# TritonDataCenter/dragnet

Measured on AMD Instinct MI355X. Metric: NDJSON records/sec (whole node), krill filter + 2-field breakdown (req.method,res.statusCode), higher is better.
Workload: dtype uint8; 1 GPU; model=dn scan: filter eq(req.method,GET) + breakdown req.method,res.statusCode, global_batch=4743501, seq_len=226, parallelism=dp1

## Files before the change

dragnet_amd/engine/gpu.py:

```python

import os
import stat
from types import SimpleNamespace

import numpy as np

from . import capacity, decode, xpose
from . import plan as planmod
from .chunks import _pad, choose_chunk_bytes, frame_files
from .decode import (
    C_DS_FAILEDEVAL, C_DS_FILTERED, C_GLOBAL_N, C_INVALID_JSON, C_LINES,
    C_OVERFLOW, C_PARSED, CM_AGG_IN, CM_BADDATE, CM_FAILEDEVAL,
    CM_FILTER_IN, CM_FILTERED, CM_N, CM_NONNUMERIC, CM_TIME_OUT, CM_UNDEF)
from .xpose import _build_xpose_layout


def _env_int(name, default):
    try:
        return int(os.environ.get(name, default))
    except ValueError:
        return default


def first_guess_slots():
# ... 287 lines not shown
    def overflowed(self):
        return int(self.counters[C_OVERFLOW].item()) > 0


    def scan_files(self, files):
        cap = self.eng.chunk_bytes
        if self._pinned is None:
            try:
                total = sum(os.stat(p).st_size for p in files)
            except OSError:
                total = 0
            cap = choose_chunk_bytes(total, cap,
                                     "DRAGNET_CHUNK_MB" in os.environ)
        pins = self._ensure_file_staging(cap)
        evs = [None, None]

        def wait(i):
            if evs[i] is not None:
                evs[i].synchronize()
                evs[i] = None

        frames = frame_files(files, [memoryview(p.numpy()) for p in pins],
                             cap, wait, _env_int("DRAGNET_READERS", 24))
        try:
            for i, n in frames:
                evs[i] = self._run_pinned(pins[i], n)
        finally:
            frames.close()

    def _ensure_file_staging(self, cap):
        torch = self.t
        if self._files is None:
            if self._pinned is None:
                self._ensure_buffers(_pad(cap))
            self._files = SimpleNamespace(
                pins=[self._pinned, torch.empty(
                    self._pinned.numel(), dtype=torch.uint8,
                    pin_memory=True)],
                copy_stream=torch.cuda.Stream(device=self.eng.device),
                dev=[self._dev_data, torch.empty_like(self._dev_data)],
                done=[torch.cuda.Event(), torch.cuda.Event()],
                idx=0)
        return self._files.pins

    def _run_pinned(self, pin, n):
        torch = self.t
        f = self._files
        padded = self._pad_pinned(pin, n)
        idx = f.idx
        f.idx ^= 1
        dev_data = f.dev[idx]
        main = torch.cuda.current_stream(self.eng.device)
        cs = f.copy_stream
        cs.wait_event(f.done[idx])
        ev = torch.cuda.Event()
        with torch.cuda.stream(cs):
            dev_data[:padded].copy_(pin[:padded], non_blocking=True)
            ev.record(cs)
        main.wait_event(ev)
        self._submit(dev_data, 0, n)
        f.done[idx].record(main)
        return ev


    def stage_resident(self, buf, n_slices=None):
        torch = self.t
        if n_slices is None:
            n_slices = _env_int("DRAGNET_SLICES", 6)
        n = len(buf)
        self._ensure_buffers(_pad(n))
        pin = self._pinned
        pin[:n] = torch.frombuffer(bytearray(buf), dtype=torch.uint8)
        padded = self._pad_pinned(pin, n)

        bounds = sorted({0, n} | {buf.rfind(b"\n", 0, n * k // n_slices) + 1
                                  for k in range(1, n_slices)})
        slices = list(zip(bounds, bounds[1:]))
        self._pool = p = SimpleNamespace(
            n=n, padded=padded, slices=slices,
            copy_stream=torch.cuda.Stream(device=self.eng.device),
            evs=[torch.cuda.Event() for _ in slices],
            dev_pp=torch.empty_like(self._dev_data),
            pass_done=[torch.cuda.Event(), torch.cuda.Event()],
            idx=0, pos=[])

        self._dev_data[:padded].copy_(pin[:padded])
        for (s, e) in slices:
            pos, nlines = self._index(self._dev_data, s, e)
            p.pos.append(
                (pos[:int(nlines.item())].clone(), nlines.clone()))

    def scan_resident(self, h2d=True):
        torch = self.t
        p = self._pool
        padded = p.padded
        dev_data = self._dev_data
        pin = self._pinned
        main = torch.cuda.current_stream(self.eng.device)
        if h2d:
            idx = p.idx
            p.idx ^= 1
            dev_data = self._dev_data if idx == 0 else p.dev_pp
            ev_done = p.pass_done[idx]
            p.copy_stream.wait_event(ev_done)
            with torch.cuda.stream(p.copy_stream):
                for k, (s, e) in enumerate(p.slices):
                    s16 = s & ~15
                    e16 = min((e + 15) & ~15, padded)
                    dev_data[s16:e16].copy_(pin[s16:e16],
                                            non_blocking=True)
                    p.evs[k].record(p.copy_stream)
        for k, (s, e) in enumerate(p.slices):
            if h2d:
                main.wait_event(p.evs[k])
                self._submit(dev_data, s, e)
            else:
                self._submit(dev_data, s, e, p.pos[k])
        if h2d:
            ev_done.record(main)


    def stage_xpose(self, buf=None):
        gran = _env_int("DRAGNET_XGRAN", 64)
        if gran not in (32, 64, 128):
            raise ValueError("DRAGNET_XGRAN must be 32, 64 or 128")
        if os.environ.get("DRAGNET_XPOSE_HOST") == "1":
            self._x = xpose.build_on_host(self.t, buf, gran,
                                          self.eng.device)
            return
        if self._pool is None:
            if buf is None:
                raise ValueError("no resident pool to transpose")
            self.stage_resident(buf)
        pos, nlines = self._index(self._dev_data, 0, self._pool.n)
        self._x = xpose.build_on_device(self.t, self.eng.ops,
                                        self._dev_data, pos, nlines, gran)

    def scan_xpose(self):
        self.state.scan_xpose(*self._x)

    def make_graph(self, h2d=True, xpose=False):
        torch = self.t

        def pass_():
            self.reset()
            if xpose:
                self.scan_xpose()
            else:
                self.scan_resident(h2d=h2d)

        try:
            pass_()
            torch.cuda.synchronize(self.eng.device)
            g = torch.cuda.CUDAGraph()
            with torch.cuda.graph(g):
                pass_()
            torch.cuda.synchronize(self.eng.device)
            return g
        except Exception:
            return None

    def reset(self):
        self.state.reset()
        if self.planner is not None:
            self.planner.occ = dict.fromkeys(self.planner.names, 0)


    def finalize(self, queries):
        return self.decode_extracted(self.extract_async(queries),
                                     queries)

    def extract_async(self, queries):
        h = self.state.extract_all()
        h["ev"] = self.t.cuda.Event()
        h["ev"].record()
        return h

    def decode_extracted(self, h, queries):
        torch = self.t
        if self._fin_stream is None:
            self._fin_stream = torch.cuda.Stream(device=self.eng.device)
        with torch.cuda.stream(self._fin_stream):
            self._fin_stream.wait_event(h["ev"])
            host = {"cnt": h["cnt"].cpu().numpy()}
            host.update(self._fetch_dicts(h))
            host["aggs"] = []
            for k_full, c_full, out_n in h["aggs"][:len(queries)]:
                n_out = min(int(out_n.item()), k_full.shape[0])
                host["aggs"].append((k_full[:n_out].cpu().numpy(),
                                     c_full[:n_out].cpu().numpy()))
        return decode.decode_snapshot(host, queries, self.cplan)

    @staticmethod
    def _fetch_dicts(h):
        n_str = int(h["n_str"].item())
        n_num = int(h["n_num"].item())
        host = {"n_str": n_str, "n_num": n_num}
        if n_str:
            host["str_off"] = h["str_off"][:n_str].cpu().numpy()
            host["str_len"] = h["str_len"][:n_str].cpu().numpy()
            used = int(h["used"].item())
            host["blob"] = h["blob"][:used].cpu().numpy()
# ... 8 lines not shown
```

dragnet_amd/ops/hip/common.h:

```cpp
#pragma once
#if defined(__HIPCC__)
#include <hip/hip_runtime.h>
#endif
#include <cstddef>
#include <cstdint>
#include "hd.h"

namespace dn {

constexpr int MAX_FIELDS = 24;
constexpr int MAX_DEPTH  = 64;
constexpr int SLOT_DEPTH = 12;
constexpr int MAX_KEY    = 8;
constexpr int MAX_SYNTH  = 8;
constexpr int PRED_STACK = 8;

enum PredOp : int32_t {
  OP_AND = 0, OP_OR = 1,
  OP_EQ = 2, OP_NE = 3, OP_LT = 4, OP_LE = 5, OP_GT = 6, OP_GE = 7,
  OP_TRUE = 8,
};

enum ConstKind : int32_t { CONST_NUM = 0, CONST_STR = 1, CONST_NULL = 2 };

// ... 22 lines not shown
enum CounterSlot : int {
  C_LINES = 0,
  C_INVALID_JSON = 1,
  C_PARSED = 2,
  C_DS_FILTERED = 3,
  C_DS_FAILEDEVAL = 4,
  C_OVERFLOW = 5,
  C_GLOBAL_N = 8,
  CM_FILTER_IN = 0, CM_FILTERED = 1, CM_FAILEDEVAL = 2,
  CM_UNDEF = 3, CM_BADDATE = 4, CM_TIME_OUT = 5,
  CM_AGG_IN = 6, CM_NONNUMERIC = 7,
  CM_N = 8,
};

constexpr uint32_t SLOT_EMPTY = 0, SLOT_CLAIMED = 1, SLOT_READY = 2;

struct AggTable {
  uint32_t* state;
  uint32_t* keys;
  double*   count;
  uint32_t  nslots;
  double*   partial;
  uint32_t  prows;
  uint32_t  pad_;
};

struct StrDict {
  uint32_t* state;
  uint64_t* hash;
  uint32_t* id;
  uint32_t* off;
  uint32_t* len;
  uint32_t  nslots;
  uint8_t*  data;
  uint32_t  data_cap;
  uint32_t* data_used;
  uint32_t* next_id;
};

struct NumDict {
  uint32_t* state;
  uint64_t* bits;
  uint32_t* id;
  uint32_t  nslots;
  uint32_t* next_id;
};


struct PlanView {
  const uint64_t* field_sigs;
  int nf;
  const int32_t* comp_slot;
  int nf_match;
  uint64_t sig_bloom;
  const int32_t* prog_nodes;
  const int32_t* prog_bounds;
  const int32_t* const_meta;
  const double*  const_dvals;
  const uint8_t* const_bytes;
  const int32_t* synth_slots;
  int ns;
  const int32_t* metric_rows;
  const int32_t* synth_req;
  const int32_t* bd_rows;
  const double*  bd_steps;
  int nm;
  int value_slot;
  int fields_slot;
  uint64_t fields_parent_sig;
};

struct ScanArgs {
  const uint8_t* data;
  const uint32_t* nl_pos;
  const uint32_t* nlines_ptr;
  uint32_t pos_cap;
  uint32_t first_start;
  uint32_t tile_cap;
  PlanView P;
  AggTable* tables;
  StrDict sdict;
  NumDict ndict;
  unsigned long long* counters;
  int data_format_skinner;
  const uint8_t* xdata;
  const unsigned long long* xwave_base;
  const uint32_t* xrec_len;
  uint32_t xn_slots;
};

}
```

dragnet_amd/ops/hip/ext.hip:

```cpp

#include <torch/extension.h>
#include <cstdlib>
#include <cstring>
#include <c10/hip/HIPStream.h>

#include "scan_kernels.hip"

namespace dn {

namespace {

#define CHECK_GPU(t) TORCH_CHECK((t).is_cuda(), #t " must be on GPU")

constexpr size_t LDS_MAX = 160 * 1024;

hipStream_t current_stream() {
  return c10::hip::getCurrentHIPStream().stream();
}

template <class... KArgs, class... Args>
void launch(const char* what, void (*kernel)(KArgs...), dim3 grid,
            dim3 block, size_t lds, Args&&... args) {
  hipLaunchKernelGGL(kernel, grid, block, lds, current_stream(),
                     std::forward<Args>(args)...);
  hipError_t err = hipGetLastError();
  TORCH_CHECK(err == hipSuccess, what, " launch failed: ",
              hipGetErrorString(err));
}

constexpr uint32_t GRID_CAP = 2048;

uint32_t grid_for(uint64_t n) {
  return (uint32_t)std::min<uint64_t>((n + BLOCK - 1) / BLOCK, GRID_CAP);
}

int env_int(const char* name, int dflt) {
  const char* v = getenv(name);
  return v ? atoi(v) : dflt;
}

size_t lds_bytes(int64_t nf, int64_t nm, int64_t ns, bool columnar) {
  return LdsLayout((int)nf, (int)nm, columnar ? 0 : (int)ns, !columnar)
      .total;
}

using ScanKernel = void (*)(ScanArgs);

ScanKernel linear_kernel(int mw) {
  switch (mw) {
    case 2: return scan_kernel_mw<2>;
    case 3: return scan_kernel_mw<3>;
    case 4: return scan_kernel_mw<4>;
    case 5: return scan_kernel_mw<5>;
    case 6: return scan_kernel_mw<6>;
    default: return scan_kernel;
  }
}

ScanKernel xpose_kernel(int mw, int xg) {
  if (xg == 32) return scan_kernel_x<4, 5>;
  if (xg == 128) return scan_kernel_x<4, 7>;
  switch (mw) {
    case 2: return scan_kernel_x<2, 6>;
    case 3: return scan_kernel_x<3, 6>;
    case 5: return scan_kernel_x<5, 6>;
    default: return scan_kernel_x<4, 6>;
  }
}

}

void newline_index(torch::Tensor data, int64_t start, int64_t n,
                   torch::Tensor seg_scratch,
                   torch::Tensor pos_out, torch::Tensor total_out) {
  CHECK_GPU(data);
  int64_t span = n - (start & ~(int64_t)15);
  uint32_t nseg = (uint32_t)((span + NL_SEG - 1) / NL_SEG);
  TORCH_CHECK((int64_t)nseg <= seg_scratch.numel(),
              "seg_scratch too small");
  if (span <= 0) {
    total_out.zero_();
    return;
  }
  const uint8_t* d = (const uint8_t*)data.data_ptr();
  uint32_t* segs = (uint32_t*)seg_scratch.data_ptr();
  uint32_t blocks = (nseg + 3) / 4;
// ... 17 lines not shown
  for (int f = 0; f < nf; f++) {
    d[f].kind = (int32_t)kinds[f];
    d[f].num = kinds[f] == COL_NUM ? (const double*)nums[f].data_ptr()
                                   : nullptr;
    d[f].soff = (kinds[f] == COL_STR || kinds[f] == COL_CODED)
                    ? (const uint32_t*)soffs[f].data_ptr()
                    : nullptr;
    d[f].slen = kinds[f] == COL_STR ? (const uint32_t*)slens[f].data_ptr()
                                    : nullptr;
  }
  return out;
}

void xpose_build(torch::Tensor data, torch::Tensor sstart,
                 torch::Tensor slen, torch::Tensor wbase,
                 int64_t n_slots, int64_t gran_log, torch::Tensor xb) {
  CHECK_GPU(data);
  CHECK_GPU(xb);
  uint32_t nw = (uint32_t)(n_slots >> 6);
  TORCH_CHECK(wbase.numel() >= (long)nw + 1, "wbase needs nw+1 rows");
  uint32_t blocks = (nw + 3) / 4;
  launch("xpose_build", xpose_build_kernel, dim3(blocks), dim3(256), 0,
         (const uint8_t*)data.data_ptr(),
         (const uint32_t*)sstart.data_ptr(),
         (const uint32_t*)slen.data_ptr(),
         (const unsigned long long*)wbase.data_ptr(),
         (uint32_t)n_slots, (int)gran_log, (uint8_t*)xb.data_ptr());
}

class ScanState {
 public:
  ScanState(py::dict plan, int64_t agg_slots, int64_t dict_slots,
            int64_t dict_data_bytes, bool dense)
      : dense_(dense) {
    auto ptr = [&](py::dict& d, const char* key) {
      owned_.push_back(py::cast<torch::Tensor>(d[key]));
      return owned_.back().data_ptr();
    };
    PlanView& P = args_.P;
    P.field_sigs = (const uint64_t*)ptr(plan, "field_sigs");
    P.nf = (int)owned_.back().numel();
    P.comp_slot = (const int32_t*)ptr(plan, "comp_slot");
    P.nf_match = py::cast<int>(plan["nf_match"]);
    P.sig_bloom = (uint64_t)py::cast<int64_t>(plan["sig_bloom"]);
    P.prog_nodes = (const int32_t*)ptr(plan, "prog_nodes");
    P.prog_bounds = (const int32_t*)ptr(plan, "prog_bounds");
    P.const_meta = (const int32_t*)ptr(plan, "const_meta");
    P.const_dvals = (const double*)ptr(plan, "const_dvals");
    P.const_bytes = (const uint8_t*)ptr(plan, "const_bytes");
    P.synth_slots = (const int32_t*)ptr(plan, "synth_slots");
    P.ns = py::cast<int>(plan["n_synth"]);
    P.metric_rows = (const int32_t*)ptr(plan, "metric_rows");
    P.nm = (int)(owned_.back().numel() / 8);
    P.synth_req = (const int32_t*)ptr(plan, "synth_req");
    P.bd_rows = (const int32_t*)ptr(plan, "bd_rows");
    P.bd_steps = (const double*)ptr(plan, "bd_steps");
    P.value_slot = py::cast<int>(plan["value_slot"]);
    P.fields_slot = py::cast<int>(plan["fields_slot"]);
    P.fields_parent_sig =
        (uint64_t)py::cast<int64_t>(plan["fields_parent_sig"]);
    args_.data_format_skinner = py::cast<bool>(plan["skinner"]) ? 1 : 0;

    for (auto& t : owned_) CHECK_GPU(t);
    device_ = owned_.front().device();

    check_slots(agg_slots, "agg table", AGG_LOG2);
    check_slots(dict_slots, "sdict", DICT_LOG2);
    check_bytes(dict_data_bytes);
    states_.resize(P.nm);
    keys_.resize(P.nm);
    counts_.resize(P.nm);
    if (dense_) partials_.resize(P.nm);
    for (int m = 0; m < P.nm; m++) alloc_agg(m, agg_slots);
    alloc_sdict(dict_slots);
    alloc_ndict(dict_slots);
    sd_data_ = zeros({dict_data_bytes}, U8);
    sd_used_ = zeros({1}, I32);
    sd_next_ = zeros({1}, I32);
    nd_next_ = zeros({1}, I32);
    counters_ = zeros({C_GLOBAL_N + P.nm * CM_N}, I64);
    bind_tables();
    bind_dicts();
    args_.counters = (unsigned long long*)counters_.data_ptr();

    int mw = env_int("DRAGNET_MIN_WAVES", 4);
    linear_ = linear_kernel(mw);
    xpose_ = xpose_kernel(mw, env_int("DRAGNET_XGRAN", 64));

    lds_ = lds_bytes(P.nf, P.nm, P.ns, false);
    TORCH_CHECK(lds_ <= LDS_MAX, "plan needs too much LDS: ", lds_);
    int tile_req = env_int("DRAGNET_LDS_STAGE", 0);
    if (tile_req != 0) {
      size_t avail = (LDS_MAX - lds_ - 256) & ~(size_t)15;
      tile_cap_ = (tile_req < 0) ? avail
                                 : std::min((size_t)tile_req, avail);
      if (tile_cap_ > 100 * 1024) tile_cap_ = 100 * 1024;
      if (tile_cap_ < 24 * 1024) tile_cap_ = 0;
    }
    args_.tile_cap = (uint32_t)tile_cap_;
  }

  void scan(torch::Tensor data, torch::Tensor nl_pos,
            torch::Tensor nlines, int64_t first_start) {
    CHECK_GPU(data);
    CHECK_GPU(nl_pos);
    ScanArgs A = args_;
    A.data = (const uint8_t*)data.data_ptr();
    A.nl_pos = (const uint32_t*)nl_pos.data_ptr();
    A.nlines_ptr = (const uint32_t*)nlines.data_ptr();
    A.pos_cap = (uint32_t)nl_pos.numel();
    A.first_start = (uint32_t)first_start;
    launch("scan_kernel", linear_, dim3(grid_for(A.pos_cap)), dim3(BLOCK),
           lds_ + tile_cap_, A);
  }

  void scan_xpose(torch::Tensor xdata, torch::Tensor wave_base,
                  torch::Tensor rec_len, int64_t n_slots) {
    CHECK_GPU(xdata);
    TORCH_CHECK(n_slots > 0, "empty transposed staging");
    ScanArgs A = args_;
    A.xdata = (const uint8_t*)xdata.data_ptr();
    A.xwave_base = (const unsigned long long*)wave_base.data_ptr();
    A.xrec_len = (const uint32_t*)rec_len.data_ptr();
    A.xn_slots = (uint32_t)n_slots;
    launch("scan_kernel_x", xpose_, dim3(grid_for(A.xn_slots)),
           dim3(BLOCK), lds_ + tile_cap_, A);
  }

  void columnar_query(torch::Tensor col_descs, torch::Tensor blob,
                      torch::Tensor values, int64_t nrows,
                      std::vector<torch::Tensor> columns) {
    ColumnLaunch L = bind_columns("columnar", col_descs, blob, values,
                                  nrows, std::move(columns));
    if (L.blocks == 0) return;
    launch("columnar_query", columnar_query_kernel, dim3(L.blocks),
           dim3(BLOCK), L.lds, L.A);
  }

  void coded_query(torch::Tensor col_descs, torch::Tensor dict_blob,
                   torch::Tensor doff, torch::Tensor dlen,
                   torch::Tensor seg_start, torch::Tensor values,
                   int64_t nrows, std::vector<torch::Tensor> columns) {
    for (auto* t : {&doff, &dlen, &seg_start}) CHECK_GPU(*t);
    TORCH_CHECK(doff.numel() == dlen.numel(), "doff / dlen differ");
    TORCH_CHECK(doff.numel() < (int64_t)0xFFFFFFFFll, "dictionary too big");
    TORCH_CHECK(seg_start.numel() >= 2 &&
                    seg_start.numel() - 1 < (int64_t)ORD_BIAS,
                "seg_start needs nfiles + 1 entries");
    ColumnLaunch L = bind_columns("coded", col_descs, dict_blob, values,
                                  nrows, std::move(columns));
    auto code2id = zeros({std::max<int64_t>(doff.numel(), 1)}, I32);
    col_inputs_.insert(col_inputs_.end(),
                       {doff, dlen, seg_start, code2id});
    CodedArgs X;
    X.ndict = (uint32_t)doff.numel();
    X.nfiles = (uint32_t)(seg_start.numel() - 1);
    X.doff = (const uint32_t*)doff.data_ptr();
    X.dlen = (const uint32_t*)dlen.data_ptr();
    X.code2id = (const uint32_t*)code2id.data_ptr();
    X.seg_start = (const uint32_t*)seg_start.data_ptr();
    if (X.ndict > 0)
      launch("dict_intern", dict_intern_kernel,
             dim3((X.ndict + 255) / 256), dim3(256), 0, L.A.sdict, L.A.blob,
             X.doff, X.dlen, X.ndict, (uint32_t*)code2id.data_ptr(),
             overflow_ptr());
    if (L.blocks == 0) return;
    launch("coded_query", coded_query_kernel, dim3(L.blocks), dim3(BLOCK),
           L.lds, L.A, X);
  }

  void reset() {
    hipStream_t st = current_stream();
    auto z = [&](torch::Tensor& t) {
      hipError_t e = hipMemsetAsync(t.data_ptr(), 0,
                                    (size_t)t.numel() * t.element_size(),
                                    st);
      TORCH_CHECK(e == hipSuccess, "reset memset failed: ",
                  hipGetErrorString(e));
    };
    for (auto& t : states_) z(t);
    for (auto& t : counts_) z(t);
    for (auto& t : partials_) z(t);
    z(sd_state_); z(sd_used_); z(sd_next_);
    z(nd_state_); z(nd_next_); z(counters_);
  }

  py::dict extract_all() {
    for (const AggTable& T : tables_) dense_reduce(T);
    const StrDict& sd = args_.sdict;
    const NumDict& nd = args_.ndict;
    py::dict out;
    out["cnt"] = counters_.clone();
    out["n_str"] = sd_next_.clone();
    out["n_num"] = nd_next_.clone();
    out["used"] = sd_used_.clone();
    out["blob"] = sd_data_.clone();

    long n_sids = std::max<long>(sd.nslots, 1);
    auto str_off = zeros({n_sids}, I32);
    auto str_len = zeros({n_sids}, I32);
    if (sd.nslots > 0)
      launch("extract_strdict", extract_strdict_kernel,
             dim3((sd.nslots + 255) / 256), dim3(256), 0, sd,
             (uint32_t*)str_off.data_ptr(), (uint32_t*)str_len.data_ptr(),
             sd.nslots);
    out["str_off"] = str_off;
    out["str_len"] = str_len;

    auto numbers = zeros({std::max<long>(nd.nslots, 1)}, F64);
// ... 45 lines not shown
  void grow_agg(int64_t m, int64_t new_slots) {
    TORCH_CHECK(!dense_, "dense tables do not grow");
    TORCH_CHECK(m >= 0 && (size_t)m < tables_.size(), "no such metric");
    AggTable old = tables_[m];
    check_slots(new_slots, "agg table", AGG_LOG2, old.nslots);
    std::vector<torch::Tensor> keep = {states_[m], keys_[m], counts_[m]};
    growing("agg" + std::to_string(m), old.nslots, new_slots,
            [&] { alloc_agg(m, new_slots); });
    bind_tables();
    launch("rehash_agg", rehash_agg_kernel, dim3((old.nslots + 255) / 256),
           dim3(256), 0, old, tables_[m], overflow_ptr());
  }

  void grow_sdict(int64_t new_slots) {
    StrDict old = args_.sdict;
    check_slots(new_slots, "sdict", DICT_LOG2, old.nslots);
    std::vector<torch::Tensor> keep = {sd_state_, sd_hash_, sd_id_,
                                       sd_off_, sd_len_};
    growing("sdict", old.nslots, new_slots, [&] { alloc_sdict(new_slots); });
    bind_dicts();
    launch("rehash_strdict", rehash_strdict_kernel,
           dim3((old.nslots + 255) / 256), dim3(256), 0, old, args_.sdict,
           overflow_ptr());
  }

  void grow_sdata(int64_t new_bytes) {
    torch::Tensor old = sd_data_;
    check_bytes(new_bytes, old.numel());
    growing("sdata", old.numel(), new_bytes,
            [&] { sd_data_ = zeros({new_bytes}, U8); });
    bind_dicts();
    hipError_t e = hipMemcpyAsync(
        sd_data_.data_ptr(), old.data_ptr(), (size_t)old.numel(),
        hipMemcpyDeviceToDevice, current_stream());
    TORCH_CHECK(e == hipSuccess, "payload copy failed: ",
                hipGetErrorString(e));
  }

  void grow_ndict(int64_t new_slots) {
    NumDict old = args_.ndict;
    check_slots(new_slots, "ndict", DICT_LOG2, old.nslots);
    std::vector<torch::Tensor> keep = {nd_state_, nd_bits_, nd_id_};
    growing("ndict", old.nslots, new_slots, [&] { alloc_ndict(new_slots); });
    bind_dicts();
    launch("rehash_numdict", rehash_numdict_kernel,
           dim3((old.nslots + 255) / 256), dim3(256), 0, old, args_.ndict,
           overflow_ptr());
  }

 private:
  static constexpr auto I32 = torch::kInt32, I64 = torch::kInt64,
                        F64 = torch::kFloat64, U8 = torch::kUInt8;

  torch::Tensor zeros(at::IntArrayRef shape, torch::ScalarType dtype) const {
    return torch::zeros(shape, torch::dtype(dtype).device(device_));
  }

  static constexpr int DICT_LOG2 = 31, AGG_LOG2 = 29;
  static void check_slots(int64_t n, const char* what, int max_log2,
                          int64_t old = 0) {
    TORCH_CHECK(n > 0 && (n & (n - 1)) == 0 && (n >> max_log2) <= 1, what,
                ": slot count must be a power of two <= 2^", max_log2);
    TORCH_CHECK(n > old, "a table may only grow (", old, " -> ", n,
                " slots)");
  }

  static void check_bytes(int64_t n, int64_t old = -1) {
    TORCH_CHECK(n <= (int64_t)0xFFFFFFFFll,
                "string payload buffer exceeds 32-bit offsets");
    TORCH_CHECK(n > old, "string payload buffer may only grow");
  }

  template <class Alloc>
  static void growing(const std::string& name, int64_t old_size,
                      int64_t new_size, Alloc&& alloc) {
    try {
      alloc();
    } catch (const c10::OutOfMemoryError& e) {
      std::string why = e.what_without_backtrace();
      TORCH_CHECK(false, "cannot grow ", name, " from ", old_size, " to ",
                  new_size, ": device allocation failed (",
                  why.substr(0, why.find('\n')), ")");
    }
  }

  struct ColumnLaunch {
    ColArgs A;
    size_t lds;
    uint32_t blocks;
  };

  ColumnLaunch bind_columns(const char* what, torch::Tensor col_descs,
                            torch::Tensor blob, torch::Tensor values,
                            int64_t nrows,
                            std::vector<torch::Tensor> columns) {
    for (auto* t : {&col_descs, &blob, &values}) CHECK_GPU(*t);
    for (auto& t : columns) {
      CHECK_GPU(t);
      TORCH_CHECK(t.numel() >= nrows, "column shorter than nrows");
    }
    TORCH_CHECK(nrows >= 0 && nrows < (int64_t)0xFFFFFFFFll, what,
                " query: row count exceeds 32 bits");
    TORCH_CHECK(values.numel() >= nrows, "values shorter than nrows");
    ColumnLaunch L;
    ColArgs& A = L.A;
    A.P = column_plan();
    TORCH_CHECK(col_descs.numel() == (int64_t)(A.P.nf * sizeof(ColDesc)),
                "col_descs does not match the plan's field count");
    L.lds = lds_bytes(A.P.nf, A.P.nm, 0, true);
    TORCH_CHECK(L.lds <= LDS_MAX, what, " plan needs too much LDS");
    A.nrows = (uint32_t)nrows;
    A.values = (const double*)values.data_ptr();
    A.blob = (const uint8_t*)blob.data_ptr();
    A.cols = (const ColDesc*)col_descs.data_ptr();
    A.tables = args_.tables;
    A.sdict = args_.sdict;
    A.ndict = args_.ndict;
    A.counters = args_.counters;
    col_inputs_ = std::move(columns);
    col_inputs_.insert(col_inputs_.end(), {col_descs, blob, values});
    L.blocks = grid_for((uint64_t)nrows);
    return L;
  }

  PlanView column_plan() const {
    PlanView P = args_.P;
    P.sig_bloom = 0;
    P.fields_parent_sig = 0;
    P.ns = 0;
    P.value_slot = -1;
    P.fields_slot = -1;
    return P;
  }

  unsigned long long* overflow_ptr() {
    return (unsigned long long*)counters_.data_ptr() + C_OVERFLOW;
  }

  void alloc_agg(size_t m, int64_t n) {
    std::tie(states_[m], keys_[m], counts_[m]) = std::make_tuple(
        zeros({n}, I32), zeros({n * MAX_KEY}, I32), zeros({n}, F64));
    if (dense_) partials_[m] = zeros({GRID_CAP, n}, F64);
  }

  void alloc_sdict(int64_t n) {
    std::tie(sd_state_, sd_hash_, sd_id_, sd_off_, sd_len_) =
        std::make_tuple(zeros({n}, I32), zeros({n}, I64), zeros({n}, I32),
                        zeros({n}, I32), zeros({n}, I32));
  }

  void alloc_ndict(int64_t n) {
    std::tie(nd_state_, nd_bits_, nd_id_) =
        std::make_tuple(zeros({n}, I32), zeros({n}, I64), zeros({n}, I32));
  }

  void bind_dicts() {
    StrDict& sd = args_.sdict;
    sd.state = (uint32_t*)sd_state_.data_ptr();
    sd.hash = (uint64_t*)sd_hash_.data_ptr();
    sd.id = (uint32_t*)sd_id_.data_ptr();
    sd.off = (uint32_t*)sd_off_.data_ptr();
    sd.len = (uint32_t*)sd_len_.data_ptr();
    sd.nslots = (uint32_t)sd_state_.numel();
    sd.data = (uint8_t*)sd_data_.data_ptr();
    sd.data_cap = (uint32_t)sd_data_.numel();
    sd.data_used = (uint32_t*)sd_used_.data_ptr();
    sd.next_id = (uint32_t*)sd_next_.data_ptr();
    NumDict& nd = args_.ndict;
    nd.state = (uint32_t*)nd_state_.data_ptr();
    nd.bits = (uint64_t*)nd_bits_.data_ptr();
    nd.id = (uint32_t*)nd_id_.data_ptr();
    nd.nslots = (uint32_t)nd_state_.numel();
    nd.next_id = (uint32_t*)nd_next_.data_ptr();
  }

  void bind_tables() {
    size_t nm = states_.size();
    tables_.resize(nm);
    for (size_t m = 0; m < nm; m++) {
      AggTable& t = tables_[m];
      t.state = (uint32_t*)states_[m].data_ptr();
      t.keys = (uint32_t*)keys_[m].data_ptr();
      t.count = (double*)counts_[m].data_ptr();
      t.nslots = (uint32_t)states_[m].numel();
      t.partial = dense_ ? (double*)partials_[m].data_ptr() : nullptr;
      t.prows = dense_ ? GRID_CAP : 0;
      t.pad_ = 0;
    }
    auto host = torch::empty({(long)(nm * sizeof(AggTable))},
                             torch::dtype(torch::kUInt8));
    memcpy(host.data_ptr(), tables_.data(), nm * sizeof(AggTable));
    table_descs_ = host.to(device_);
    args_.tables = (AggTable*)table_descs_.data_ptr();
  }

  static void dense_reduce(const AggTable& T) {
    if (T.partial == nullptr || T.prows == 0) return;
    uint32_t tiles = (T.nslots + 15) / 16;
    uint32_t splits = 32;
    while (splits > 1 && T.prows / splits < 16) splits /= 2;
    uint32_t rows_per_blk = (T.prows + splits - 1) / splits;
    rows_per_blk = (rows_per_blk + 3) & ~3u;
    launch("mfma_reduce", mfma_reduce_kernel, dim3(tiles, splits),
           dim3(64), 0, T, rows_per_blk);
  }

  std::vector<torch::Tensor> states_, keys_, counts_, partials_, owned_;
  std::vector<torch::Tensor> col_inputs_;
  torch::Tensor sd_state_, sd_hash_, sd_id_, sd_off_, sd_len_;
  torch::Tensor sd_data_, sd_used_, sd_next_;
  torch::Tensor nd_state_, nd_bits_, nd_id_, nd_next_;
  torch::Tensor counters_, table_descs_;
  c10::Device device_ = c10::kCPU;
  const bool dense_;
  ScanArgs args_ = {};
  std::vector<AggTable> tables_;
  ScanKernel linear_ = nullptr, xpose_ = nullptr;
  size_t lds_ = 0, tile_cap_ = 0;
};

}

PYBIND11_MODULE(TORCH_EXTENSION_NAME, m) {
  m.doc() = "dragnet_amd MI355X scan engine (gfx950 HIP kernels)";
  m.def("newline_index", &dn::newline_index, "device-side newline index");
  m.def("xpose_build", &dn::xpose_build, "device-side wave transpose");
  m.def("col_descs_host", &dn::col_descs_host);
  m.def("lds_bytes", &dn::lds_bytes, py::arg("nf"), py::arg("nm"),
        py::arg("ns") = 0, py::arg("columnar") = false,
        "dynamic LDS bytes of a scan / columnar launch (host only)");
  py::class_<dn::ScanState>(m, "ScanState")
      .def(py::init<py::dict, int64_t, int64_t, int64_t, bool>(),
           py::kw_only(), py::arg("plan"), py::arg("agg_slots"),
           py::arg("dict_slots"), py::arg("dict_data_bytes"),
           py::arg("dense"))
      .def("scan", &dn::ScanState::scan, py::arg("data"),
           py::arg("nl_pos"), py::arg("nlines"), py::arg("first_start"),
           "fused NDJSON scan over one chunk")
      .def("scan_xpose", &dn::ScanState::scan_xpose, py::arg("xdata"),
           py::arg("wave_base"), py::arg("rec_len"), py::arg("n_slots"))
      .def("columnar_query", &dn::ScanState::columnar_query,
           py::arg("col_descs"), py::arg("blob"), py::arg("values"),
           py::arg("nrows"), py::arg("columns"),
           "K7: query over uploaded index columns")
      .def("coded_query", &dn::ScanState::coded_query,
           py::arg("col_descs"), py::arg("dict_blob"), py::arg("doff"),
           py::arg("dlen"), py::arg("seg_start"), py::arg("values"),
           py::arg("nrows"), py::arg("keep"),
           "query over merged dictionary-coded sidecar columns")
      .def("reset", &dn::ScanState::reset)
      .def("extract_all", &dn::ScanState::extract_all)
      .def("occupancy", &dn::ScanState::occupancy,
           "device int64 [ready slots per metric..., string ids, "
           "payload bytes, number ids]")
      .def("sizes", &dn::ScanState::sizes)
      .def_property_readonly("counters", &dn::ScanState::counters)
      .def("grow_agg", &dn::ScanState::grow_agg, py::arg("metric"),
           py::arg("new_slots"),
           "rehash one metric's table into a larger zeroed one")
      .def("grow_sdict", &dn::ScanState::grow_sdict, py::arg("new_slots"))
      .def("grow_sdata", &dn::ScanState::grow_sdata, py::arg("new_bytes"))
      .def("grow_ndict", &dn::ScanState::grow_ndict, py::arg("new_slots"));
  m.attr("MAX_KEY") = (int)dn::MAX_KEY;
  m.attr("MAX_FIELDS") = (int)dn::MAX_FIELDS;
}
```

dragnet_amd/ops/hip/scan_kernels.hip:

```cpp

#include "common.h"
#include <hip/hip_runtime.h>

extern "C++" {
#include "scan_text.h"
#include "scan_record.h"
#include "scan_tables.h"

namespace dn {

typedef double dn_d4 __attribute__((ext_vector_type(4)));

__global__ void mfma_reduce_kernel(AggTable T, uint32_t rows_per_blk) {
  uint32_t slot0 = blockIdx.x * 16;
  uint32_t r0 = blockIdx.y * rows_per_blk;
  uint32_t r1 = r0 + rows_per_blk;
  if (r1 > T.prows) r1 = T.prows;
  int l = threadIdx.x;
  uint32_t n = slot0 + (l & 15);
  dn_d4 acc = {0.0, 0.0, 0.0, 0.0};
  const double* P = T.partial;
  size_t stride = T.nslots;
  for (uint32_t rt = r0; rt < r1; rt += 4) {
    uint32_t rr = rt + (uint32_t)(l >> 4);
// ... 263 lines not shown
        bool sok = true;
        for (int k = 0; k < M[3]; k++) {
          int si = P.synth_req[M[4] + k];
          uint32_t ok = (synth_ok >> (2 * si)) & 3u;
          if (ok != 1) {
            atomicAdd(&mc[ok == 2 ? CM_UNDEF : CM_BADDATE], 1ull);
            sok = false; break;
          }
        }
        if (!sok) continue;

        if (M[5]) {
          int si = P.synth_req[M[4] + M[3] - 1];
          double ts = synth_val_at(si);
          if (!(ts >= (double)M[6] && ts < (double)M[7])) {
            atomicAdd(&mc[CM_TIME_OUT], 1ull); continue;
          }
        }

        atomicAdd(&mc[CM_AGG_IN], 1ull);

        uint32_t key[MAX_KEY];
        int nk = M[1];
        bool drop = false, overflow = false;
        for (int bi = 0; bi < nk; bi++) {
          const int32_t* B = &P.bd_rows[(M[2] + bi) * 4];
          double step = P.bd_steps[M[2] + bi];
          uint8_t t; double num = 0.0; uint32_t so = 0, sl = 0;
          if (B[0] == 1) {
            int si = B[1];
            if (((synth_ok >> (2 * si)) & 3u) == 1) {
              t = T_NUM; num = synth_val_at(si);
            } else t = T_MISSING;
          } else {
            int slot = B[1];
            int cs2 = P.comp_slot[slot];
            if (cs2 >= 0 && fv.get_type(cs2) != T_MISSING)
              slot = cs2;
            t = fv.get_type(slot);
            num = fv.get_num(slot);
            so = fv.get_soff(slot); sl = fv.get_slen(slot);
          }
          uint32_t code;
          if (!encode_key_col(A.sdict, A.ndict, BV, t, num, so, sl, B[2],
                              step, code, drop, overflow))
            break;
#pragma unroll
          for (int kk = 0; kk < MAX_KEY; kk++)
            if (kk == bi) key[kk] = code;
        }
        if (overflow) { atomicAdd(&lcnt[C_OVERFLOW], 1ull); continue; }
        if (drop) { atomicAdd(&mc[CM_NONNUMERIC], 1ull); continue; }
#pragma unroll
        for (int k = 0; k < MAX_KEY; k++)
          if (k >= nk) key[k] = 0;

        uint64_t kh = agg_key_hash(m, key);

        if (!A.data_format_skinner) {
          uint64_t unproc = __ballot(true);
          bool leader = false;
          double wsum = 0.0;
          while (unproc) {
            int src = (int)(__ffsll((long long)unproc) - 1);
            uint64_t src_kh = __shfl(kh, src);
            bool same = (kh == src_kh);
            uint64_t grp = __ballot(same);
            if (same && __lane_id() == src) {
              leader = true;
              wsum = (double)__popcll(grp);
            }
            unproc &= ~grp;
          }
          if (!leader) continue;
          weight = wsum;
        }
        lds_cache_add<1>(cache, A.tables, A.counters, lcnt, m, key, nk, kh,
                      weight);
      }
    }
  }
}

template <int XP>
DEV void scan_kernel_body(char* smem, ScanArgs A) {
  const PlanView& P = A.P;
  const int nf = P.nf;

  const LdsLayout L(nf, P.nm, P.ns, true);
  LdsCacheEntry* cache = reinterpret_cast<LdsCacheEntry*>(smem + L.cache);
  unsigned long long* lcnt =
      reinterpret_cast<unsigned long long*>(smem + L.lcnt);
  const int NCNT = C_GLOBAL_N + P.nm * CM_N;
  double* synth_lds = reinterpret_cast<double*>(smem + L.synth);
  uint64_t* sig_lds = reinterpret_cast<uint64_t*>(smem + L.sig);
  uint8_t* tile = reinterpret_cast<uint8_t*>(smem + L.tile);
  block_agg_init(cache, lcnt, NCNT);

  FV fv;
  fv.type = reinterpret_cast<uint8_t*>(smem + L.fv_type);
  fv.soff = reinterpret_cast<uint32_t*>(smem + L.fv_soff);
  fv.slen = reinterpret_cast<uint32_t*>(smem + L.fv_slen);
  fv.tid = threadIdx.x;

  if constexpr (XP != 0) {
    const uint32_t stride_x = gridDim.x * BLOCK;
    for (uint32_t rbase = blockIdx.x * BLOCK; rbase < A.xn_slots;
         rbase += stride_x) {
      uint32_t r = rbase + threadIdx.x;
      if (r < A.xn_slots) {
        uint32_t len = A.xrec_len[r];
        if (len != 0xFFFFFFFFu) {
          XBytesT<XP> BV;
          BV.base = A.xdata + A.xwave_base[r >> 6]
                    + ((size_t)(r & 63u) << XP);
          process_record(BV, 0u, len, A, P, fv, lcnt, cache, sig_lds,
                         synth_lds);
        }
      }
    }
  } else {
  uint32_t nlines = *A.nlines_ptr;
  if (nlines > A.pos_cap) nlines = A.pos_cap;
  const uint32_t stride = gridDim.x * BLOCK;
  for (uint32_t rbase = blockIdx.x * BLOCK; rbase < nlines;
       rbase += stride) {
    uint32_t r = rbase + threadIdx.x;
    bool active = r < nlines;

    Bytes BV;
    BV.mem = A.data;
    BV.bias = 0;
    uint32_t t_start = rbase ? A.nl_pos[rbase - 1] + 1 : A.first_start;
    uint32_t r_last = rbase + BLOCK - 1;
    if (r_last >= nlines) r_last = nlines - 1;
    uint32_t t_end = A.nl_pos[r_last] + 1;
    uint32_t t_base = t_start & ~15u;
    uint32_t span = t_end - t_base;
    bool staged = A.tile_cap >= 16 && span <= A.tile_cap;
    if (staged) {
      const uint4* g16 = reinterpret_cast<const uint4*>(A.data + t_base);
      uint4* l16 = reinterpret_cast<uint4*>(tile);
      uint32_t n16 = (span + 15) >> 4;
      for (uint32_t i = threadIdx.x; i < n16; i += BLOCK)
        l16[i] = g16[i];
      __syncthreads();
      BV.mem = tile;
      BV.bias = t_base;
    }

    if (active) {
      uint32_t start = r ? A.nl_pos[r - 1] + 1 : A.first_start;
      uint32_t end = A.nl_pos[r];
      process_record(BV, start, end, A, P, fv, lcnt, cache, sig_lds,
                     synth_lds);
    }

    if (staged) __syncthreads();
  }
  }

  block_agg_flush(cache, lcnt, NCNT, P, A.tables, A.counters);
}


__global__ void extract_agg_kernel(AggTable T, uint32_t* out_keys,
                                   double* out_counts, uint32_t* out_n,
                                   uint32_t max_out) {
  uint32_t s = blockIdx.x * blockDim.x + threadIdx.x;
  if (s >= T.nslots) return;
  if (atomic_load_relaxed(&T.state[s]) != SLOT_READY) return;
  uint32_t i = atomicAdd(out_n, 1u);
  if (i >= max_out) return;
  for (int k = 0; k < MAX_KEY; k++)
    out_keys[i * MAX_KEY + k] = T.keys[s * MAX_KEY + k];
  out_counts[i] = T.count[s];
}

__global__ void extract_strdict_kernel(StrDict D, uint32_t* out_off,
                                       uint32_t* out_len, uint32_t max_ids) {
  uint32_t s = blockIdx.x * blockDim.x + threadIdx.x;
  if (s >= D.nslots) return;
  if (atomic_load_relaxed(&D.state[s]) != SLOT_READY) return;
  uint32_t id = D.id[s];
  if (id >= max_ids) return;
  out_off[id] = D.off[s];
  out_len[id] = D.len[s];
}

__global__ void extract_numdict_kernel(NumDict D, double* out_vals,
                                       uint32_t max_ids) {
  uint32_t s = blockIdx.x * blockDim.x + threadIdx.x;
  if (s >= D.nslots) return;
  if (atomic_load_relaxed(&D.state[s]) != SLOT_READY) return;
  uint32_t id = D.id[s];
  if (id >= max_ids) return;
  out_vals[id] = __longlong_as_double(
      (long long)atomic_load_relaxed(&D.bits[s]));
}

}

#include "scan_rehash.h"

#include "scan_columns.h"

}
```

dragnet_amd/ops/hip/scan_tables.h:

```cpp
#pragma once
#include "scan_record.h"

namespace dn {

#define DEV __device__ __forceinline__

constexpr int LDS_CACHE = 128;

template <typename T>
DEV T atomic_load_relaxed(const T* p) {
  return __hip_atomic_load(p, __ATOMIC_RELAXED, __HIP_MEMORY_SCOPE_AGENT);
}
template <typename T>
DEV void atomic_store_relaxed(T* p, T v) {
  __hip_atomic_store(p, v, __ATOMIC_RELAXED, __HIP_MEMORY_SCOPE_AGENT);
}
DEV void drain_stores() {
  asm volatile("s_waitcnt vmcnt(0)" ::: "memory");
}


template <class BS>
DEV uint64_t hash_bytes(BS BV, uint32_t off, uint32_t len) {
  uint64_t h = FNV_OFFSET;
// ... 111 lines not shown
      if (st == SLOT_EMPTY) {
        uint32_t prev = atomicCAS(&T.state[s], SLOT_EMPTY, SLOT_CLAIMED);
        if (prev == SLOT_EMPTY) {
#pragma unroll
          for (int k = 0; k < MAX_KEY; k++)
            atomic_store_relaxed(&T.keys[s * MAX_KEY + k],
                                 k < nk ? key[k] : 0u);
          drain_stores();
          atomic_store_relaxed(&T.state[s], SLOT_READY);
          atomicAdd(&T.count[s], w);
          return true;
        }
        continue;
      }
      __builtin_amdgcn_s_sleep(1);
    }
  }
  return false;
}

DEV uint32_t agg_insert_slot(const AggTable& T, const uint32_t* key,
                             int nk) {
  uint64_t h = agg_table_hash(key, nk);
  uint32_t mask = T.nslots - 1;
  uint32_t s = (uint32_t)h & mask;
  uint32_t max_probes = 256;
  for (uint32_t probes = 0; probes < max_probes; probes++, s = (s + 1) & mask) {
    while (true) {
      uint32_t st = atomic_load_relaxed(&T.state[s]);
      if (st == SLOT_READY) {
        bool same = true;
#pragma unroll
        for (int k = 0; k < MAX_KEY; k++)
          if (k < nk &&
              atomic_load_relaxed(&T.keys[s * MAX_KEY + k]) != key[k])
            same = false;
        if (same) return s;
        break;
      }
      if (st == SLOT_EMPTY) {
        uint32_t prev = atomicCAS(&T.state[s], SLOT_EMPTY, SLOT_CLAIMED);
        if (prev == SLOT_EMPTY) {
#pragma unroll
          for (int k = 0; k < MAX_KEY; k++)
            atomic_store_relaxed(&T.keys[s * MAX_KEY + k],
                                 k < nk ? key[k] : 0u);
          drain_stores();
          atomic_store_relaxed(&T.state[s], SLOT_READY);
          return s;
        }
        continue;
      }
      __builtin_amdgcn_s_sleep(1);
    }
  }
  return 0xFFFFFFFFu;
}

DEV bool agg_add(const AggTable& T, const uint32_t* key, int nk,
                 double w, unsigned long long* gflag) {
  if (T.partial != nullptr) {
    if (atomic_load_relaxed(gflag) != 0ull) return false;
    uint32_t s = agg_insert_slot(T, key, nk);
    if (s == 0xFFFFFFFFu) {
      atomicAdd(gflag, 1ull);
      return false;
    }
    atomicAdd(&T.partial[(size_t)(blockIdx.x % T.prows) * T.nslots + s],
              w);
    return true;
  }
  return agg_insert(T, key, nk, w);
}


struct LdsCacheEntry {
  uint64_t hash;
  uint32_t metric;
  uint32_t key[MAX_KEY];
  double count;
};

struct LdsLayout {
  size_t fv_soff, fv_slen, fv_type, cache, lcnt, synth, sig, tile, total;
  __host__ __device__ __forceinline__
  LdsLayout(int nf, int nm, int ns, bool parse_state) {
    size_t off = 0;
    fv_soff = off; off += (size_t)nf * BLOCK * sizeof(uint32_t);
    fv_slen = off; off += (size_t)nf * BLOCK * sizeof(uint32_t);
    fv_type = off; off += (size_t)nf * BLOCK * sizeof(uint8_t);
    off = (off + 15) & ~(size_t)15;
    cache = off; off += (size_t)LDS_CACHE * sizeof(LdsCacheEntry);
    lcnt = off;
    off += (size_t)(C_GLOBAL_N + nm * CM_N) * sizeof(unsigned long long);
    synth = sig = off;
    if (parse_state) {
      off += (size_t)ns * BLOCK * sizeof(double);
      sig = off; off += (size_t)SIG_DEPTH * BLOCK * sizeof(uint64_t);
    }
    off = (off + 15) & ~(size_t)15;
    tile = off;
    total = off + 64;
  }
};


template <class BS>
DEV bool encode_key_col(const StrDict& sdict, const NumDict& ndict, BS BV,
                       uint8_t t, double num, uint32_t so, uint32_t sl,
                       int bucket, double step, uint32_t& code,
                        bool& drop, bool& overflow) {
  if (bucket != BUCKET_NONE) {
    if (t == T_STR) {
      num = js_to_number(BV, so, sl);
      if (!(num == num) || num == __builtin_inf() ||
          num == -__builtin_inf())
        { drop = true; return false; }
      t = T_NUM;
    }
    if (t != T_NUM || !finite_num(num)) { drop = true; return false; }
    double ordf = bucket_ordinal(bucket, num, step);
    if (ord_is_small(ordf)) {
      code = make_code(TAG_ORD, (uint32_t)((int)ordf + ORD_BIAS));
    } else {
      uint32_t id = intern_number(ndict, ordf);
      if (id == 0xFFFFFFFFu) { overflow = true; return false; }
      code = make_code(TAG_NUM, id);
    }
  } else if (t == T_MISSING) {
    code = make_code(TAG_SPECIAL, SPECIAL_UNDEF);
  } else if (t == T_NULL) {
    code = make_code(TAG_SPECIAL, SPECIAL_NULL);
  } else if (t == T_TRUE) {
    code = make_code(TAG_SPECIAL, SPECIAL_TRUE);
  } else if (t == T_FALSE) {
    code = make_code(TAG_SPECIAL, SPECIAL_FALSE);
  } else if (t == T_OBJ) {
    code = make_code(TAG_SPECIAL, SPECIAL_OBJECT);
  } else if (t == T_ARR) {
    uint32_t id = intern_string(sdict, BV, so, sl);
    if (id == 0xFFFFFFFFu || id >= (1u << 27)) { overflow = true; return false; }
    code = make_code(TAG_SPECIAL, SPECIAL_ARRJSON | (id << 3));
  } else if (t == T_NUM) {
    uint32_t id = intern_number(ndict, num);
    if (id == 0xFFFFFFFFu) { overflow = true; return false; }
    code = make_code(TAG_NUM, id);
  } else {
    uint32_t id = intern_string(sdict, BV, so, sl);
    if (id == 0xFFFFFFFFu) { overflow = true; return false; }
    code = make_code(TAG_STR, id);
  }
  return true;
}

DEV uint64_t agg_key_hash(int m, const uint32_t* key) {
  uint64_t kh = mix64((uint64_t)m * 0x9E3779B97F4A7C15ull + 1);
  for (int k = 0; k < MAX_KEY; k++) kh = mix64(kh ^ key[k]);
  return kh == 0 ? 1 : kh;
}

template <int UNROLL>
DEV void lds_cache_add(LdsCacheEntry* cache, AggTable* tables,
                       unsigned long long* counters,
                       unsigned long long* lcnt, int m,
                       const uint32_t* key, int nk, uint64_t kh,
                       double weight) {
  bool cached = false;
  uint32_t ci = (uint32_t)kh & (LDS_CACHE - 1);
#pragma unroll UNROLL
  for (int attempt = 0; attempt < 8; attempt++) {
    unsigned long long prev = atomicCAS(
        (unsigned long long*)&cache[ci].hash, 0ull,
        (unsigned long long)kh);
    if (prev == 0) {
      cache[ci].metric = m;
      for (int k = 0; k < MAX_KEY; k++) cache[ci].key[k] = key[k];
      atomicAdd(&cache[ci].count, weight);
      cached = true;
      break;
    }
    if (prev == (unsigned long long)kh && cache[ci].metric == m) {
      bool same = true;
      for (int k = 0; k < MAX_KEY; k++)
        if (cache[ci].key[k] != key[k]) { same = false; break; }
      if (same) {
// ... 45 lines not shown
```

Baseline: 248.9 million records/s.

## Use persistent grid with atomic tile claiming and single resident-pool scan launch

Scan kernels now use dynamic work distribution. Each block claims BLOCK-sized tiles from a global atomic counter instead of a fixed grid-stride loop, and the grid is capped at the number of blocks that can be resident at once, from an occupancy query. The last block to finish resets the counter. Separately, the resident no-H2D path now concatenates per-slice newline positions and issues one launch instead of one per slice. This is meant to reduce load imbalance from variable-length records and cut launch overhead. In exchange it adds a per-tile atomic plus a barrier, and the counter is shared between launches, so kernels running concurrently on different streams could interfere.

```diff
diff --git a/dragnet_amd/engine/gpu.py b/dragnet_amd/engine/gpu.py
--- a/dragnet_amd/engine/gpu.py
+++ b/dragnet_amd/engine/gpu.py
@@ -393,42 +393,41 @@
             evs=[torch.cuda.Event() for _ in slices],
             dev_pp=torch.empty_like(self._dev_data),
             pass_done=[torch.cuda.Event(), torch.cuda.Event()],
-            idx=0, pos=[])
+            idx=0, pos_all=None)
 
         self._dev_data[:padded].copy_(pin[:padded])
+        pos_parts, counts = [], []
         for (s, e) in slices:
             pos, nlines = self._index(self._dev_data, s, e)
-            p.pos.append(
-                (pos[:int(nlines.item())].clone(), nlines.clone()))
+            pos_parts.append(pos[:int(nlines.item())].clone())
+            counts.append(nlines.clone())
+        p.pos_all = (torch.cat(pos_parts),
+                     torch.cat(counts).sum(dtype=torch.int32).reshape(1))
 
     def scan_resident(self, h2d=True):
         torch = self.t
         p = self._pool
+        if not h2d:
+            self._submit(self._dev_data, 0, p.n, p.pos_all)
+            return
         padded = p.padded
-        dev_data = self._dev_data
         pin = self._pinned
         main = torch.cuda.current_stream(self.eng.device)
-        if h2d:
-            idx = p.idx
-            p.idx ^= 1
-            dev_data = self._dev_data if idx == 0 else p.dev_pp
-            ev_done = p.pass_done[idx]
-            p.copy_stream.wait_event(ev_done)
-            with torch.cuda.stream(p.copy_stream):
-                for k, (s, e) in enumerate(p.slices):
-                    s16 = s & ~15
-                    e16 = min((e + 15) & ~15, padded)
-                    dev_data[s16:e16].copy_(pin[s16:e16],
-                                            non_blocking=True)
-                    p.evs[k].record(p.copy_stream)
+        idx = p.idx
+        p.idx ^= 1
+        dev_data = self._dev_data if idx == 0 else p.dev_pp
+        ev_done = p.pass_done[idx]
+        p.copy_stream.wait_event(ev_done)
+        with torch.cuda.stream(p.copy_stream):
+            for k, (s, e) in enumerate(p.slices):
+                s16 = s & ~15
+                e16 = min((e + 15) & ~15, padded)
+                dev_data[s16:e16].copy_(pin[s16:e16], non_blocking=True)
+                p.evs[k].record(p.copy_stream)
         for k, (s, e) in enumerate(p.slices):
-            if h2d:
-                main.wait_event(p.evs[k])
-                self._submit(dev_data, s, e)
-            else:
-                self._submit(dev_data, s, e, p.pos[k])
-        if h2d:
-            ev_done.record(main)
+            main.wait_event(p.evs[k])
+            self._submit(dev_data, s, e)
+        ev_done.record(main)
 
 
     def stage_xpose(self, buf=None):
diff --git a/dragnet_amd/ops/hip/common.h b/dragnet_amd/ops/hip/common.h
--- a/dragnet_amd/ops/hip/common.h
+++ b/dragnet_amd/ops/hip/common.h
@@ -128,6 +128,7 @@
   StrDict sdict;
   NumDict ndict;
   unsigned long long* counters;
+  uint32_t* claim;
   int data_format_skinner;
   const uint8_t* xdata;
   const unsigned long long* xwave_base;
diff --git a/dragnet_amd/ops/hip/ext.hip b/dragnet_amd/ops/hip/ext.hip
--- a/dragnet_amd/ops/hip/ext.hip
+++ b/dragnet_amd/ops/hip/ext.hip
@@ -1,7 +1,9 @@
 
 #include <torch/extension.h>
+#include <algorithm>
 #include <cstdlib>
 #include <cstring>
+#include <ATen/hip/impl/HIPGuardImplMasqueradingAsCUDA.h>
 #include <c10/hip/HIPStream.h>
 
 #include "scan_kernels.hip"
@@ -185,6 +187,8 @@
     bind_tables();
     bind_dicts();
     args_.counters = (unsigned long long*)counters_.data_ptr();
+    claim_ = zeros({2}, I32);
+    args_.claim = (uint32_t*)claim_.data_ptr();
 
     int mw = env_int("DRAGNET_MIN_WAVES", 4);
     linear_ = linear_kernel(mw);
@@ -201,6 +205,11 @@
       if (tile_cap_ < 24 * 1024) tile_cap_ = 0;
     }
     args_.tile_cap = (uint32_t)tile_cap_;
+    resident_linear_ = resident_blocks("scan_kernel", linear_);
+    resident_xpose_ = resident_blocks("scan_kernel_x", xpose_);
+    int grid_req = env_int("DRAGNET_SCAN_GRID", 0);
+    if (grid_req != 0)
+      grid_override_ = (uint32_t)std::clamp(grid_req, 1, (int)GRID_CAP);
   }
 
   void scan(torch::Tensor data, torch::Tensor nl_pos,
@@ -213,7 +222,8 @@
     A.nlines_ptr = (const uint32_t*)nlines.data_ptr();
     A.pos_cap = (uint32_t)nl_pos.numel();
     A.first_start = (uint32_t)first_start;
-    launch("scan_kernel", linear_, dim3(grid_for(A.pos_cap)), dim3(BLOCK),
+    launch("scan_kernel", linear_,
+           dim3(scan_grid(A.pos_cap, resident_linear_)), dim3(BLOCK),
            lds_ + tile_cap_, A);
   }
 
@@ -226,8 +236,9 @@
     A.xwave_base = (const unsigned long long*)wave_base.data_ptr();
     A.xrec_len = (const uint32_t*)rec_len.data_ptr();
     A.xn_slots = (uint32_t)n_slots;
-    launch("scan_kernel_x", xpose_, dim3(grid_for(A.xn_slots)),
-           dim3(BLOCK), lds_ + tile_cap_, A);
+    launch("scan_kernel_x", xpose_,
+           dim3(scan_grid(A.xn_slots, resident_xpose_)), dim3(BLOCK),
+           lds_ + tile_cap_, A);
   }
 
   void columnar_query(torch::Tensor col_descs, torch::Tensor blob,
@@ -439,6 +450,24 @@
                   new_size, ": device allocation failed (",
                   why.substr(0, why.find('\n')), ")");
     }
+  }
+
+  uint32_t resident_blocks(const char* what, ScanKernel kernel) const {
+    int per_cu = 0, cus = 0;
+    c10::hip::HIPGuardMasqueradingAsCUDA on_device(device_);
+    hipError_t e = hipOccupancyMaxActiveBlocksPerMultiprocessor(
+        &per_cu, kernel, BLOCK, lds_ + tile_cap_);
+    if (e == hipSuccess)
+      e = hipDeviceGetAttribute(&cus, hipDeviceAttributeMultiprocessorCount,
+                                device_.index());
+    TORCH_CHECK(e == hipSuccess && per_cu > 0 && cus > 0, what,
+                " occupancy query failed: ", hipGetErrorString(e));
+    return (uint32_t)per_cu * (uint32_t)cus;
+  }
+
+  uint32_t scan_grid(uint64_t n, uint32_t resident) const {
+    if (grid_override_) return grid_override_;
+    return std::min(grid_for(n), resident);
   }
 
   struct ColumnLaunch {
@@ -567,13 +596,15 @@
   torch::Tensor sd_state_, sd_hash_, sd_id_, sd_off_, sd_len_;
   torch::Tensor sd_data_, sd_used_, sd_next_;
   torch::Tensor nd_state_, nd_bits_, nd_id_, nd_next_;
-  torch::Tensor counters_, table_descs_;
+  torch::Tensor counters_, table_descs_, claim_;
   c10::Device device_ = c10::kCPU;
   const bool dense_;
   ScanArgs args_ = {};
   std::vector<AggTable> tables_;
   ScanKernel linear_ = nullptr, xpose_ = nullptr;
   size_t lds_ = 0, tile_cap_ = 0;
+  uint32_t resident_linear_ = 0, resident_xpose_ = 0;
+  uint32_t grid_override_ = 0;
 };
 
 }
diff --git a/dragnet_amd/ops/hip/scan_kernels.hip b/dragnet_amd/ops/hip/scan_kernels.hip
--- a/dragnet_amd/ops/hip/scan_kernels.hip
+++ b/dragnet_amd/ops/hip/scan_kernels.hip
@@ -369,6 +369,25 @@
   }
 }
 
+
+DEV uint32_t tiles_of(uint32_t n) {
+  return n / BLOCK + (n % BLOCK != 0);
+}
+
+DEV uint32_t claim_tile(uint32_t* claim, uint32_t* lds_words, uint32_t nth) {
+  uint32_t* w = &lds_words[nth & 1u];
+  if (threadIdx.x == 0) *w = atomicAdd(&claim[0], 1u);
+  __syncthreads();
+  return __builtin_amdgcn_readfirstlane(*w);
+}
+
+DEV void claim_leave(uint32_t* claim) {
+  if (threadIdx.x == 0 && atomicAdd(&claim[1], 1u) == gridDim.x - 1) {
+    atomic_store_relaxed(&claim[0], 0u);
+    atomic_store_relaxed(&claim[1], 0u);
+  }
+}
+
 template <int XP>
 DEV void scan_kernel_body(char* smem, ScanArgs A) {
   const PlanView& P = A.P;
@@ -390,10 +409,15 @@
   fv.slen = reinterpret_cast<uint32_t*>(smem + L.fv_slen);
   fv.tid = threadIdx.x;
 
+  uint32_t* claim_lds =
+      reinterpret_cast<uint32_t*>(smem + L.claim + A.tile_cap);
+  uint32_t claims = 0;
+
   if constexpr (XP != 0) {
-    const uint32_t stride_x = gridDim.x * BLOCK;
-    for (uint32_t rbase = blockIdx.x * BLOCK; rbase < A.xn_slots;
-         rbase += stride_x) {
+    const uint32_t ntiles = tiles_of(A.xn_slots);
+    uint32_t tile_no;
+    while ((tile_no = claim_tile(A.claim, claim_lds, claims++)) < ntiles) {
+      uint32_t rbase = tile_no * BLOCK;
       uint32_t r = rbase + threadIdx.x;
       if (r < A.xn_slots) {
         uint32_t len = A.xrec_len[r];
@@ -409,9 +433,10 @@
   } else {
   uint32_t nlines = *A.nlines_ptr;
   if (nlines > A.pos_cap) nlines = A.pos_cap;
-  const uint32_t stride = gridDim.x * BLOCK;
-  for (uint32_t rbase = blockIdx.x * BLOCK; rbase < nlines;
-       rbase += stride) {
+  const uint32_t ntiles = tiles_of(nlines);
+  uint32_t tile_no;
+  while ((tile_no = claim_tile(A.claim, claim_lds, claims++)) < ntiles) {
+    uint32_t rbase = tile_no * BLOCK;
     uint32_t r = rbase + threadIdx.x;
     bool active = r < nlines;
 
@@ -448,6 +473,7 @@
   }
 
   block_agg_flush(cache, lcnt, NCNT, P, A.tables, A.counters);
+  claim_leave(A.claim);
 }
 
 
diff --git a/dragnet_amd/ops/hip/scan_tables.h b/dragnet_amd/ops/hip/scan_tables.h
--- a/dragnet_amd/ops/hip/scan_tables.h
+++ b/dragnet_amd/ops/hip/scan_tables.h
@@ -217,7 +217,8 @@
 };
 
 struct LdsLayout {
-  size_t fv_soff, fv_slen, fv_type, cache, lcnt, synth, sig, tile, total;
+  size_t fv_soff, fv_slen, fv_type, cache, lcnt, synth, sig, tile, total,
+      claim;
   __host__ __device__ __forceinline__
   LdsLayout(int nf, int nm, int ns, bool parse_state) {
     size_t off = 0;
@@ -236,6 +237,7 @@
     off = (off + 15) & ~(size_t)15;
     tile = off;
     total = off + 64;
+    claim = total - 8;
   }
 };
 
```

New measurement: 248.7 million records/s (median of 3 runs). Within noise of the previous version (-0.1%).
